# kuldeepbrd1/graspLDM

Measured on AMD Instinct MI355X. Metric: grasps/sec whole-node (1024-pt cloud, 100 DDIM steps), higher is better.
Workload: dtype f32 (GEMMs as split-f16 x3 partial products on the f16 matrix pipe, f32 accumulation; GroupNorm / LayerNorm / attention / scheduler in f32); 1 GPU; LDM mode, 256 synthetic 1024-pt clouds per GPU x 20 grasps, 100 DDIM steps: BASELINE.json configs[2] per GPU (configs[3] = this per-GPU workload on 8 GPUs); experiment=fpc, clouds_per_gpu=256, grasps_per_cloud=20, points=1024, ddim_steps=100, encoder=PVCNNEncoder (shipped fpc config), parallelism=cloud-sharded x1, weights=synthetic recipe seed 0, streams=3

## Files before the change

### graspldm_amd/_lib.py

```python
import ctypes
import os

_PKG = os.path.dirname(os.path.abspath(__file__))
LIB_PATH = os.environ.get("GLDM_LIB") or os.path.join(_PKG, "libgldm_hip.so")

ABI_VERSION = 10


class GldmError(RuntimeError):
    pass


_lib = None

_ll = ctypes.c_longlong
_ull = ctypes.c_ulonglong
_vp, _i, _f = ctypes.c_void_p, ctypes.c_int, ctypes.c_float

_SIGNATURES = {
    "gldm_ball_query": [_vp, _vp, _i, _i, _i, _f, _i, _vp, _vp],
    "gldm_grouping_forward": [_vp, _vp, _i, _i, _i, _i, _i, _vp, _vp],
    "gldm_gather_features_forward": [_vp, _vp, _i, _i, _i, _i, _vp, _vp],
    "gldm_furthest_point_sampling": [_vp, _i, _i, _i, _vp, _vp],
    "gldm_three_nn_interpolate_forward": [_vp, _vp, _vp, _i, _i, _i, _i, _vp, _vp, _vp, _vp],
    "gldm_avg_voxelize_forward": [_vp, _vp, _i, _i, _i, _i, _vp, _vp, _vp, _vp],
    "gldm_trilinear_devoxelize_forward": [_vp, _vp, _i, _i, _i, _i, _i, _vp, _vp, _vp, _vp],
    "gldm_voxel_coords": [_vp, _i, _i, _i, _i, _f, _vp, _vp, _vp],
    "gldm_farthest_points_euclid": [_vp, _i, _i, _i, _vp, _vp],
    "gldm_normalize_cloud": [_vp, _i, _i, _f, _f, _f, _f, _f, _f, _vp, _vp, _vp],
    "gldm_gather_points": [_vp, _vp, _i, _i, _i, _vp, _vp],
    "gldm_sa_group": [_vp, _vp, _vp, _i, _i, _i, _i, _f, _i, _vp, _vp, _vp],
    "gldm_r1d_cond_embed": [_vp, _vp, _vp, _i, _i, _i, _i, _vp, _vp],
    "gldm_denoise": [_vp, _vp, _vp, _vp, _i, _vp, _i, _vp, _vp, _i, _i, _i, _vp, _vp, _vp, _vp, _vp, _vp],
    "gldm_denoise_rng": [_vp, _vp, _vp, _vp, _i, _vp, _i, _vp, _i, _i, _vp, _ull, _ll, _vp, _vp, _vp, _vp],
    "gldm_step_noise_rng": [_ull, _ll, _i, _i, _i, _vp, _vp],
    "gldm_decode": [_vp, _vp, _vp, _i, _vp, _i, _vp, _vp, _vp, _vp],
    "gldm_pose_epilogue": [_vp, _vp, _vp, _vp, _i, _i, _i, _vp, _vp, _vp, _vp],
    "gldm_conv3d_k3": [_vp, _vp, _vp, _i, _i, _i, _i, _vp, _vp, _vp],
    "gldm_conv3d_k3_cl": [_vp, _vp, _vp, _i, _i, _i, _i, _vp, _vp, _vp],
    "gldm_conv3d_k3_generic": [_vp, _vp, _vp, _i, _i, _i, _i, _vp, _vp, _vp],
    "gldm_conv3d_k3_f16x2": [_vp, _vp, _vp, _i, _i, _i, _i, _vp, _vp, _vp],
    "gldm_conv3d_k3_f16x2_gn": [_vp, _vp, _vp, _vp, _i, _i, _i, _i, _vp, _vp, _i, _vp],
    "gldm_groupnorm_coef": [_vp, _vp, _vp, _i, _i, _i, _i, _f, _vp, _vp],
    "gldm_gn_swish_chan_sum": [_vp, _vp, _i, _i, _i, _vp, _vp],
    "gldm_gn_swish_chan_sum_cl": [_vp, _vp, _i, _i, _i, _vp, _vp],
    "gldm_se_gate_parts": [_vp, _i, _vp, _vp, _i, _i, _i, _i, _i, _vp, _vp],
    "gldm_groupnorm_swish": [_vp, _vp, _vp, _vp, _i, _i, _i, _i, _f, _vp, _vp],
    "gldm_se_gate": [_vp, _vp, _vp, _i, _i, _i, _i, _i, _vp, _vp],
    "gldm_bias_act": [_vp, _vp, _i, _i, ctypes.c_longlong, _i, _vp],
    "gldm_devoxelize_fused": [_vp, _vp, _vp, _vp, _i, _i, _i, _i, _vp, _vp],
    "gldm_devoxelize_gn_fused": [_vp, _vp, _vp, _vp, _vp, _i, _i, _i, _i, _vp, _vp],
    "gldm_devoxelize_gn_cl_fused": [_vp, _vp, _vp, _vp, _vp, _i, _i, _i, _i, _vp, _vp],
    "gldm_pointwise_mlp": [_vp, _vp, _vp, _i, _i, _i, _i, _i, _vp, _vp, _i, _vp, _vp, _vp],
    "gldm_pointwise_mlp2": [_vp, _vp, _vp, _i, _vp, _vp, _i, _i, _i, _i, _vp, _vp, _i, _vp, _vp, _vp],
    "gldm_pointwise_small": [_vp, _vp, _vp, _i, _i, _i, ctypes.c_longlong, _i, _vp, _vp],
    "gldm_pointwise_any": [_vp, _vp, _vp, _i, _i, _i, ctypes.c_longlong, _i, _vp, _vp],
    "gldm_linear_rows": [_vp, _vp, _vp, _i, _i, _i, _vp, _vp],
    "gldm_pointwise_mlp_f16x2": [_vp, _vp, _vp, _i, _i, _i, _i, _i, _vp, _vp, _i, _vp, _vp, _vp],
    "gldm_row_max": [_vp, _ll, _i, _vp, _vp],
    "gldm_pointwise_mlp_f16x2_pm": [_vp, _vp, _vp, _i, _i, _i, _i, _i, _vp, _vp],
    "gldm_pointwise_mlp_f16x2_add": [_vp, _vp, _vp, _vp, _ll, _ll, _ll, _i, _i, _i, _i, _i, _vp, _vp],
    "gldm_pointwise_mlp2_f16x2": [_vp, _vp, _vp, _i, _vp, _vp, _i, _i, _i, _i, _vp, _vp, _i, _vp, _vp, _vp, _vp],
    "gldm_sa_mlp_forward": [_vp, _vp, _vp, _vp, _vp, _i, _i, _i, _i, _i, _i, _vp, _vp, _vp, _vp, _vp, _vp],
    "gldm_sa_mlp_forward_f16x2": [_vp, _vp, _vp, _vp, _vp, _i, _i, _i, _i, _i, _i, _vp, _vp, _vp, _vp, _vp, _vp, _vp],
    "gldm_sa_mlp_forward_f16x2_pre": [_vp, _vp, _vp, _i, _vp, _vp, _i, _i, _i, _i, _i, _i, _vp, _vp, _vp, _vp, _vp, _vp, _vp],
}


# ... 61 lines not shown
```

### graspldm_amd/csrc/resnet1d.hip

```cpp
#include <hip/hip_runtime.h>
#include <type_traits>
#include <stdint.h>
#include <stdio.h>
#include <stdlib.h>

#include "gldm.h"
#include "wstream.h"
#include "devstate.h"

#define GLDM_API extern "C" __attribute__((visibility("default")))

#ifdef GLDM_DEBUG_KNOBS
#define GLDM_SKIP(c, bit) ((c).skip & (bit))
#define GLDM_STAMPS(p) (p)
#else
#define GLDM_SKIP(c, bit) false
#define GLDM_STAMPS(p) ((long long *)nullptr)
#endif

namespace {

using f32x4 = __attribute__((ext_vector_type(4))) float;
typedef __attribute__((address_space(3))) float lds_f;
typedef __attribute__((address_space(3))) f32x4 lds_f4;

constexpr int kHeads = 4, kDimHead = 32, kHidden = kHeads * kDimHead;
constexpr int kMaxC = 256;
constexpr int kMaxSegs = 64;

template <int NC>
struct Geo {
  static constexpr int kWaves = NC / 8;
  static constexpr int kThreads = kWaves * 64;
// ... 363 lines not shown
}


typedef __attribute__((ext_vector_type(8))) _Float16 f16x8;

__device__ __forceinline__ void split_planes8(const float (&x)[8], u32x4 (&pl)[kSplit]) {
#pragma unroll
  for (int q = 0; q < 4; ++q) {
    unsigned h, l;
    split_f16x2(x[2 * q], x[2 * q + 1], h, l);
    pl[0][q] = h;
    pl[1][q] = l;
  }
}
__device__ __forceinline__ f32x4 mfma_h(const u32x4 &a, const u32x4 &b, const f32x4 &c) {
  return __builtin_amdgcn_mfma_f32_16x16x32_f16(__builtin_bit_cast(f16x8, a), __builtin_bit_cast(f16x8, b), c, 0, 0, 0);
}
__device__ __forceinline__ f32x4 mfma_split(const u32x4 (&a)[kSplit], const u32x4 (&b)[kSplit], f32x4 acc) {
  acc = mfma_h(a[0], b[1], acc);
  acc = mfma_h(a[1], b[0], acc);
  return mfma_h(a[0], b[0], acc);
}

#if defined(GLDM_DEBUG_KNOBS) && defined(GLDM_EXP_NO_A)
constexpr bool kExpNoA = true;
#else
constexpr bool kExpNoA = false;
#endif
#if defined(GLDM_DEBUG_KNOBS) && defined(GLDM_EXP_NO_B)
constexpr bool kExpNoB = true;
#else
constexpr bool kExpNoB = false;
#endif
struct NoPreA { static constexpr bool on = false; };
template <int MT>
struct PreA {
  static constexpr bool on = true;
  static constexpr int kSets = MT == 1 ? 3 : 1;
  u32x4 a[kSets][MT][kSplit];
  __device__ __forceinline__ void request(const WStream &wv, int mt0, int cin) {
    const int kb32 = cin >> 5, kblocks = 3 * kb32;
#pragma unroll
    for (int t = 0; t < kSets; ++t)
#pragma unroll
      for (int mi = 0; mi < MT; ++mi)
#pragma unroll
        for (int pl = 0; pl < kSplit; ++pl) a[t][mi][pl] = wv.raw_at(((mt0 + mi) * kblocks + t * kb32) * kFragBytes, pl * 1024);
  }
};

template <int MT, int P0, int NP, class PRE = NoPreA>
__device__ __forceinline__ void gemm_pm3_pl(const Ctx &c, const float *__restrict__ wp3, int cin, int mt0,
                                            const float *planes, f32x4 (&acc)[MT][NP], const PRE &pre = PRE()) {
  constexpr int PB0 = P0 > 0 ? P0 - 1 : 0, PB1 = P0 + NP < 4 ? P0 + NP : 3, NB = PB1 - PB0 + 1;
  const int col = c.lane & 15, g = c.lane >> 4;
  const int kb32 = cin >> 5, kblocks = 3 * kb32;
  const WStream wv(wp3, c.lane);
  const lds_u4 *pl3 = (const lds_u4 *)planes + g * 64 + 16 * PB0 + col;
  constexpr int NA = MT == 1 ? 3 : 2;
  constexpr int NBUF = (MT == 1 && NB <= 3) ? 2 : 1;
  u32x4 a[NA][MT][kSplit];
  u32x4 bs[NBUF][NB][kSplit];
  auto load_a = [&](int buf, int t, int kb) {
    if (kExpNoA && kb > 0) return;
#pragma unroll
    for (int mi = 0; mi < MT; ++mi)
#pragma unroll
      for (int pl = 0; pl < kSplit; ++pl)
        a[buf][mi][pl] = wv.raw_at(((mt0 + mi) * kblocks + t * kb32 + kb) * kFragBytes, pl * 1024);
  };
  auto load_b = [&](int buf, int kb) {
    if (kExpNoB && kb > 0) return;
#pragma unroll
    for (int q = 0; q < NB; ++q)
#pragma unroll
      for (int pl = 0; pl < kSplit; ++pl) bs[buf][q][pl] = pl3[(kb * kSplit + pl) * 256 + 16 * q];
  };
  auto tap_mfmas = [&](int abuf, int bbuf, int t) {
#pragma unroll
    for (int mi = 0; mi < MT; ++mi)
// ... 131 lines not shown
        for (int st = 0; st < 6; ++st) step(st, kb0);
      }
    }
  } else {
    static_assert(MT == 1 || NT == 4, "two m-tiles per wave: all four tiles");
    u32x4 bs[2][kSplit];
    auto load_b1 = [&](int buf, int kb, int t, int q) {
#pragma unroll
      for (int pl = 0; pl < kSplit; ++pl) bs[buf][pl] = pl3[(kb * kSplit + pl) * G::kPlaneU4 + 16 * q + 4 * t];
    };
    first_a();
    load_b1(0, 0, 0, 0);
    auto step = [&](int st, int kb0) {
      const int t = st % 3, kb = kb0 + st / 3;
      const int nt = (st + 1) % 3, nkb0 = kb0 + (st + 1) / 3, nkb = nkb0 < last ? nkb0 : last;
      load_a((st + 1) & 1, nt, nkb);
#pragma unroll
      for (int q = 0; q < 4; ++q) {
        if (q < 3) load_b1((q + 1) & 1, kb, t, q + 1);
        else load_b1(0, nkb, nt, 0);
        __builtin_amdgcn_sched_barrier(0);
#pragma unroll
        for (int mi = 0; mi < MT; ++mi) acc[mi][q] = mfma_split(a[st & 1][mi], bs[q & 1], acc[mi][q]);
        __builtin_amdgcn_sched_barrier(0);
      }
    };
    for (int kb0 = 0; kb0 < kb32; kb0 += 2) {
#pragma unroll
      for (int st = 0; st < 6; ++st) step(st, kb0);
    }
  }
}

struct NoFirst { static constexpr bool on = false; };
struct Frag3 { static constexpr bool on = true; u32x4 p[kSplit]; };
template <int KB32, int MT, int NT, class PRE = NoPre, int MS = 1, int LL = 4, class FIRST = NoFirst>
__device__ __forceinline__ void gemm1_pl(const Ctx &c, const float *__restrict__ wp3, int mt0, int nt0, const float *planes,
                                         f32x4 (&acc)[MT][NT], const PRE &pre = PRE(), const FIRST &first = FIRST()) {
  const int col = c.lane & 15, g = c.lane >> 4;
  const WStream wv(wp3, c.lane);
  using PGx = PG<LL>;
  const lds_u4 *pl3 = (const lds_u4 *)planes + g * PGx::kCols + PGx::kOff + 16 * nt0 + col;
  u32x4 a[2][MT][kSplit];
  u32x4 bs[2][kSplit];
  auto load_a = [&](int buf, int kb) {
#pragma unroll
    for (int mi = 0; mi < MT; ++mi) {
      const int sb = ((mt0 + mi * MS) * KB32 + kb) * kFragBytes;
#pragma unroll
      for (int pl = 0; pl < kSplit; ++pl) a[buf][mi][pl] = wv.raw_at(sb, pl * 1024);
    }
  };
  auto load_b = [&](int buf, int kb, int ni) {
#pragma unroll
    for (int pl = 0; pl < kSplit; ++pl) bs[buf][pl] = pl3[(kb * kSplit + pl) * PGx::kPlaneU4 + 16 * ni];
  };
  if constexpr (FIRST::on) {
#pragma unroll
    for (int pl = 0; pl < kSplit; ++pl) a[0][0][pl] = first.p[pl];
    if constexpr (MT > 1) {
#pragma unroll
      for (int mi = 1; mi < MT; ++mi) {
        const int sb = ((mt0 + mi * MS) * KB32) * kFragBytes;
#pragma unroll
        for (int pl = 0; pl < kSplit; ++pl) a[0][mi][pl] = wv.raw_at(sb, pl * 1024);
      }
    }
  } else {
    load_a(0, 0);
  }
  load_b(0, 0, 0);
  __builtin_amdgcn_sched_barrier(0);
  pre();
  __builtin_amdgcn_sched_barrier(0);
#pragma unroll
  for (int kb = 0; kb < KB32; ++kb) {
    if (kb + 1 < KB32) load_a((kb + 1) & 1, kb + 1);
    __builtin_amdgcn_sched_barrier(0);
#pragma unroll
    for (int ni = 0; ni < NT; ++ni) {
      const int step = kb * NT + ni, nxt = step + 1;
      if (nxt < KB32 * NT) load_b(nxt & 1, nxt / NT, nxt % NT);
      __builtin_amdgcn_sched_barrier(0);
#pragma unroll
      for (int mi = 0; mi < MT; ++mi) acc[mi][ni] = mfma_split(a[kb & 1][mi], bs[step & 1], acc[mi][ni]);
      __builtin_amdgcn_sched_barrier(0);
    }
  }
}

// ... 327 lines not shown
  const int sm = LL == 16 ? (c.lane & 3) : cl;
  f32x4 acc[MT][NP];
  const bool has_ss = FIN == 1 && g.ss_w >= 0;
  const bool ss_tab = LL == 16 && has_ss && c.ss_lane != nullptr;
  const int ekb = g.E >> 4;
  const WStream wss(c.w + (has_ss ? g.ss_w : 0), c.lane);
  f32x4 ga[MT], be[MT], sc[MT], sh[MT], a_sc[MT], a_sh[MT];
  auto load_params = [&]() {
#pragma unroll
    for (int mi = 0; mi < MT; ++mi) {
      const int mt = mt0 + mi, row0 = 16 * mt + 4 * kq;
      ga[mi] = *reinterpret_cast<const f32x4 *>(c.w + g.gamma_off + row0);
      be[mi] = *reinterpret_cast<const f32x4 *>(c.w + g.beta_off + row0);
      sc[mi] = f32x4{1.f, 1.f, 1.f, 1.f};
      sh[mi] = f32x4{0.f, 0.f, 0.f, 0.f};
      if (ss_tab) {
        sc[mi] = *reinterpret_cast<const f32x4 *>(c.ss_lane + g.tab_off + row0);
        sh[mi] = *reinterpret_cast<const f32x4 *>(c.ss_lane + g.tab_off + g.C + row0);
      } else if (has_ss) {
        const float *sb = c.w + g.ss_b;
        sc[mi] = *reinterpret_cast<const f32x4 *>(sb + row0);
        sh[mi] = *reinterpret_cast<const f32x4 *>(sb + g.C + row0);
        a_sc[mi] = wss[(size_t)mt * ekb * 64];
        a_sh[mi] = wss[(size_t)((g.C >> 4) + mt) * ekb * 64];
      }
    }
  };
  lds_f *hsc = (lds_f *)(c.lds + GG::kMiscHs);
  float hs = 1.0f;
  if constexpr (FIN == 2) hs = hsc[sm];
#pragma unroll
  for (int mi = 0; mi < MT; ++mi) {
    f32x4 bv = f32x4{0.f, 0.f, 0.f, 0.f};
    if (bias) bv = *reinterpret_cast<const f32x4 *>(bias + 16 * (mt0 + mi) + 4 * kq);
    if constexpr (FIN == 2) {
      const float hinv = __builtin_amdgcn_rcpf(hs);
#pragma unroll
      for (int r = 0; r < 4; ++r) bv[r] *= hinv;
    }
#pragma unroll
    for (int p = 0; p < NP; ++p) acc[mi][p] = bv;
  }
  GLDM_WV_STAMP(c, 0, (long long)__builtin_readcyclecounter());
  GLDM_WV_STAMP(c, 3, (long long)(cin * 1000 + cout));
  const bool src_is_x = src == c.lds + GG::kBufX;
  const float *bplanes = c.lds + (cin > kPlaneMaxC ? PGx::kW : (src_is_x ? PGx::kX : PGx::kH));
  if constexpr (LL == 16) gemm_sm3_pl<MT, P0, NP, PRE>(c, wp, cin, mt0, bplanes, acc, pre);
  else gemm_pm3_pl<MT, P0, NP, PRE>(c, wp, cin, mt0, bplanes, acc, pre);
  GLDM_WV_STAMP(c, 1, (long long)__builtin_readcyclecounter());
  if (FIN != 0) load_params();
  constexpr bool kWide = MT == 2;
  constexpr bool kPark = kWide && LL == 16;
  f32x4 *pk = reinterpret_cast<f32x4 *>(c.park) + (size_t)(c.wave * MT * NP) * 64 + c.lane;
  f32x4 parked[FIN == 2 && kPark ? MT : 1][FIN == 2 && kPark ? NP : 1];
  if constexpr (FIN == 2 && kPark) {
#pragma unroll
    for (int mi = 0; mi < MT; ++mi)
#pragma unroll
      for (int p = 0; p < NP; ++p) parked[mi][p] = pk[(mi * NP + p) * 64];
  }
  hook();
  if constexpr (FIN == 0) {
    if (alias) __syncthreads();
    if (live) {
      lds_f *d3 = (lds_f *)dst;
#pragma unroll
      for (int mi = 0; mi < MT; ++mi)
// ... 347 lines not shown
#pragma unroll
    for (int co = 0; co < 4; ++co) {
      float acc = cw.b[co];
#pragma unroll
      for (int ci = 0; ci < 4; ++ci) {
        const f32x4 wr = cw.wt[4 * ci + co];
        acc += wr[0] * lft[ci];
        acc += wr[1] * in[ci];
        acc += wr[2] * rgt[ci];
      }
      out[co] = acc;
    }
  };
  auto gn_act = [&](float (&v)[4], const ConvW &cw, bool ss) {
#pragma unroll
    for (int co = 0; co < 4; ++co) {
      const float m = half_sum(row_pair_sum(v[co])) * 0.25f;
      const float d = v[co] - m;
      const float rs = __builtin_amdgcn_rsqf(half_sum(row_pair_sum(d * d)) * 0.25f + 1e-5f);
      float y = d * rs * cw.g[co] + cw.be[co];
      if (ss) y = y * sc[co] + sh[co];
      v[co] = silu(y);
    }
  };
  float y[4], z[4];
  conv3(x, k1, y);
  gn_act(y, k1, true);
  conv3(y, k2, z);
  gn_act(z, k2, false);
#pragma unroll
  for (int co = 0; co < 4; ++co) X[pswz(co, n)] = x[co] + z[co];
}

template <int NT, int NPW, bool FULL, int LL = 4, class FIRST = NoFirst>
__device__ __forceinline__ void out_ln_wave(const Ctx &c, const float *wp, const float *bias, int mt0, int nt0,
                                            bool active, int p0, const float *src, int cin, float *xres, int C,
                                            const float *gain, const FIRST &first = FIRST()) {
  using GG = Geo<64>;
  constexpr int NC = 64;
  const int kq = c.lane >> 4, col = c.lane & 15;
  f32x4 acc[1][NT];
  lds_f *red1 = (lds_f *)(c.lds + GG::kMiscRed1), *red2 = (lds_f *)(c.lds + GG::kMiscRed2);
  const int row0 = 16 * mt0 + 4 * kq;
  const int nloc = C < 16 ? C : 16;
  f32x4 gv = f32x4{0.f, 0.f, 0.f, 0.f};
  if (active) {
    const f32x4 bv = *reinterpret_cast<const f32x4 *>(bias + row0);
#pragma unroll
    for (int ni = 0; ni < NT; ++ni) acc[0][ni] = bv;
    gemm1_pl<kHidden / 32, 1, NT, NoPre, 1, LL, FIRST>(c, wp, mt0, nt0, c.lds + PG<LL>::kH, acc, NoPre(), first);
    gv = *reinterpret_cast<const f32x4 *>(gain + row0);
    const float inv_n = __builtin_amdgcn_rcpf((float)nloc);
#pragma unroll
    for (int ni = 0; ni < NT; ++ni) {
      float s1 = 0.f;
#pragma unroll
      for (int r = 0; r < 4; ++r) s1 += (FULL || row0 + r < C) ? acc[0][ni][r] : 0.f;
      s1 = half_sum(row_pair_sum(s1));
      const float ml = s1 * inv_n;
      float s2 = 0.f;
#pragma unroll
      for (int r = 0; r < 4; ++r) {
        const float d = (FULL || row0 + r < C) ? acc[0][ni][r] - ml : 0.f;
        s2 += d * d;
      }
      s2 = half_sum(row_pair_sum(s2));
      if (kq == 0) {
        red1[c.wave * NC + 16 * (nt0 + ni) + col] = s1;
        red2[c.wave * NC + 16 * (nt0 + ni) + col] = s2;
      }
    }
  }
  __syncthreads();
  if (active) {
    const float inv_c = __builtin_amdgcn_rcpf((float)C), inv_n = __builtin_amdgcn_rcpf((float)nloc);
    lds_f *x3 = (lds_f *)xres;
#pragma unroll
    for (int ni = 0; ni < NT; ++ni) {
      const int cc = 16 * (nt0 + ni) + col;
      float ps[NPW], pm[NPW], tot = 0.f;
#pragma unroll
      for (int q = 0; q < NPW; ++q) {
        ps[q] = red1[(p0 + q) * NC + cc];
        pm[q] = red2[(p0 + q) * NC + cc];
// ... 47 lines not shown

template <int RP>
__device__ __forceinline__ void column_stats8(const Ctx &c, const float *src, float inv_c) {
  constexpr int NC = 64;
  using GG = Geo<NC>;
  const lds_f *s3 = (const lds_f *)src;
  const int n = 8 * c.wave + (c.lane & 7), rp = c.lane >> 3;
  float v[RP], sum = 0.f;
#pragma unroll
  for (int i = 0; i < RP; ++i) {
    v[i] = s3[pswz(rp + 8 * i, n)];
    sum += v[i];
  }
  auto all_parts = [](float x) {
    x += dpp_mov<0x128>(x);
    return half_sum(row_pair_sum(x));
  };
  const float mean = all_parts(sum) * inv_c;
  float m2 = 0.f;
#pragma unroll
  for (int i = 0; i < RP; ++i) {
    const float d = v[i] - mean;
    m2 = fmaf(d, d, m2);
  }
  const float rstd = __builtin_amdgcn_rsqf(all_parts(m2) * inv_c + 1e-5f);
  if (rp == 0) {
    ((lds_f *)(c.lds + GG::kMiscRed1))[n] = mean;
    ((lds_f *)(c.lds + GG::kMiscRed2))[n] = rstd;
  }
}

constexpr int kAttExch = 512 * 64;
static_assert(kAttExch + 8 * 24 * 16 <= Geo<64>::kArena, "attention exchange slots");
template <int KB32>
__device__ __forceinline__ void qkv_att_pm(const Ctx &c, int w_off, int s_off, const float *src, int C) {
  constexpr int NC = 64;
  using GG = Geo<NC>;
  if (GLDM_SKIP(c, 8)) return;
  const int head = c.wave >> 1, half = c.wave & 1;
  const int mt0 = 2 * head + half;
  const int sm = c.lane & 15, kq = c.lane >> 4;
  f32x4 acc[3][4];
  if constexpr (KB32 == 0) {
    const int n = c.lane;
    const lds_f *s3 = (const lds_f *)src;
    float x[4];
#pragma unroll
    for (int ci = 0; ci < 4; ++ci) x[ci] = s3[pswz(ci, n)];
    const float mean = (x[0] + x[1] + x[2] + x[3]) * 0.25f;
    float vt = 0.f;
#pragma unroll
    for (int ci = 0; ci < 4; ++ci) {
      const float d = x[ci] - mean;
      vt += d * d;
    }
    const float rstd = __builtin_amdgcn_rsqf(vt * 0.25f + 1e-5f);
    lds_f *ysc = (lds_f *)(c.lds + GG::kMiscRed1);
#pragma unroll
    for (int k = 0; k < 4; ++k) ysc[64 * k + n] = (x[k] - mean) * rstd;
    const WStream wv(c.w + w_off, c.lane);
    f32x4 f[3];
#pragma unroll
    for (int t = 0; t < 3; ++t) f[t] = wv[(size_t)(mt0 + 8 * t) * 64];
    float b[4];
#pragma unroll
    for (int j = 0; j < 4; ++j) b[j] = ysc[64 * kq + 16 * j + sm];
#pragma unroll
    for (int t = 0; t < 3; ++t)
#pragma unroll
      for (int j = 0; j < 4; ++j)
        acc[t][j] = __builtin_amdgcn_mfma_f32_16x16x4f32(f[t][0], b[j], f32x4{0.f, 0.f, 0.f, 0.f}, 0, 0, 0);
  } else {
    const float *wp = c.w + w_off, *srow = c.w + s_off;
    f32x4 sv[3];
#pragma unroll
    for (int mi = 0; mi < 3; ++mi) sv[mi] = *reinterpret_cast<const f32x4 *>(srow + 16 * (mt0 + 8 * mi) + 4 * kq);
#pragma unroll
    for (int mi = 0; mi < 3; ++mi)
#pragma unroll
      for (int ni = 0; ni < 4; ++ni) acc[mi][ni] = f32x4{0.f, 0.f, 0.f, 0.f};
    const float inv_c = __builtin_amdgcn_rcpf((float)C);
    auto stats = [&]() { column_stats8<4 * KB32>(c, src, inv_c); };
    gemm1_pl<KB32, 3, 4, decltype(stats), 8>(c, wp, mt0, 0, c.lds + kPlaneX, acc, stats);
    __syncthreads();
    const lds_f *mean3 = (const lds_f *)(c.lds + GG::kMiscRed1), *rstd3 = (const lds_f *)(c.lds + GG::kMiscRed2);
#pragma unroll
    for (int ni = 0; ni < 4; ++ni) {
      const float rstd = rstd3[16 * ni + sm];
      const float mr = mean3[16 * ni + sm] * rstd;
#pragma unroll
      for (int mi = 0; mi < 3; ++mi)
#pragma unroll
        for (int r = 0; r < 4; ++r) acc[mi][ni][r] = acc[mi][ni][r] * rstd - mr * sv[mi][r];
    }
  }
  float kn[4][4];
#pragma unroll
  for (int r = 0; r < 4; ++r) {
    const float km = fmaxf(fmaxf(acc[1][0][r], acc[1][1][r]), fmaxf(acc[1][2][r], acc[1][3][r]));
    float ks = 0.f;
#pragma unroll
    for (int p = 0; p < 4; ++p) {
      kn[p][r] = fast_exp(acc[1][p][r] - km);
      ks += kn[p][r];
    }
    const float inv = __builtin_amdgcn_rcpf(ks);
#pragma unroll
    for (int p = 0; p < 4; ++p) kn[p][r] *= inv;
  }
  float qe[4][4], qm[4], qs[4];
#pragma unroll
  for (int p = 0; p < 4; ++p) {
    float m = fmaxf(fmaxf(acc[0][p][0], acc[0][p][1]), fmaxf(acc[0][p][2], acc[0][p][3]));
    m = half_max(row_pair_max(m));
    float sum = 0.f;
#pragma unroll
// ... 731 lines not shown
  for (int i = 0; i < 4; ++i) sv[i] = *reinterpret_cast<const f32x4 *>(srow + 16 * mtile(i) + 4 * g);
  const float svv[2] = {srow[16 * mtile(4) + p], srow[16 * mtile(5) + p]};
  __syncthreads();
  const lds_f *mean3 = (const lds_f *)(c.lds + GG::kMiscRed1), *rstd3 = (const lds_f *)(c.lds + GG::kMiscRed2);
  constexpr float kL2e = 1.44269504088896340736f;
#pragma unroll
  for (int e = 0; e < 2; ++e) {
    const int sm = s0 + e;
    {
      const float rstd = rstd3[4 * p + sm];
      const float mr = mean3[4 * p + sm] * rstd;
#pragma unroll
      for (int i = 0; i < 4; ++i)
#pragma unroll
        for (int r = 0; r < 4; ++r) acc[i][e][r] = (acc[i][e][r] * rstd - mr * sv[i][r]) * kL2e;
    }
#pragma unroll
    for (int r = 0; r < 4; ++r) {
      const float rstd = rstd3[4 * (4 * g + r) + sm];
      const float mr = mean3[4 * (4 * g + r) + sm] * rstd;
      acc[4][e][r] = acc[4][e][r] * rstd - mr * svv[0];
      acc[5][e][r] = acc[5][e][r] * rstd - mr * svv[1];
    }
    const f32x4 qa[2] = {acc[0][e], acc[1][e]}, ka[2] = {acc[2][e], acc[3][e]}, vt[2] = {acc[4][e], acc[5][e]};
    f32x4 o[2];
    quad16_attention_head(qa, ka, vt, o);
#pragma unroll
    for (int u = 0; u < 2; ++u)
      store_planes4<16>(c.lds + PGx::kH, kDimHead * h + 16 * u + 4 * g, 4 * p + sm, o[u][0], o[u][1], o[u][2], o[u][3]);
  }
  __syncthreads();
}


template <int NC, int L>
__device__ __forceinline__ void run_tape(const Ctx &c0, const gldm_r1d_desc &d, const int *tape, kernarg_int *ktape, int n_ops, int E, long long *stamps) {
#if defined(GLDM_DEBUG_KNOBS) && defined(GLDM_EXP_LDS_TAPE)
  constexpr bool KARG = false;
#else
  constexpr bool KARG = NC == 64;
#endif
  for (int op = 0; op < n_ops; ++op) {
    if (stamps && c0.tid == 0) stamps[op] = (long long)__builtin_readcyclecounter();
    Ctx c = c0;
    asm volatile("" : "+v"(c.tid), "+v"(c.lane));
    int o[kOpInts];
    read_op<KARG>(tape, ktape, op, o);
    if (o[0] == OP_CONV && o[5] * o[6] >= 128 * 128) __builtin_amdgcn_s_setprio(0);
    else __builtin_amdgcn_s_setprio(3);
    switch (o[0]) {
      case OP_CONV: {
        if constexpr (NC == 64) {
          if (o[7] & kFlagFused) {
            int q[kOpInts];
            read_op<KARG>(tape, ktape, op + 1, q);
            const GnEpilogue g1{1, o[8], o[9], o[10], o[11], E, o[6], o[6] / 4, c.lds + o[4], (o[7] >> kFlagTabShift) << 2};
            const GnEpilogue g2{2, q[8], q[9], -1, 0, E, q[6], q[6] / 4, c.lds + q[4], 0};
            resblock_pm<L == 16 ? 16 : 4>(c, o[1], o[2], q[1], q[2], c.lds + o[3], c.lds + o[4], o[6], g1, g2, stamps ? stamps + op + 1 : nullptr);
            ++op;
            break;
          }
        }
        const int mode = GLDM_SKIP(c, 1) ? 0 : (o[7] >> 9) & 3;
        const GnEpilogue g{mode, o[8], o[9], GLDM_SKIP(c, 16) ? -1 : o[10], o[11], E, o[6], o[6] / 4, c.lds + o[4],
                           (o[7] >> kFlagTabShift) << 2};
        conv_gemm<NC, L>(c, o[1], o[2], c.lds + o[3], o[5], o[7] & 255, c.lds + o[4], o[6], (o[7] & kFlagAlias) != 0, 0, g);
        break;
      }
      case OP_QUAD:
        if constexpr (NC == 64 && L == 4) {
          if (c.wave < 4)
            quad_narrow_levels(c, (kernarg_desc *)((__attribute__((address_space(4))) const char *)__builtin_amdgcn_kernarg_segment_ptr() +
                                                    offsetof(RunArgs, d)));
#if defined(GLDM_DEBUG_KNOBS) && defined(GLDM_QEXP_DUP)
          else if (GLDM_QEXP_DUP == 2)
            quad_narrow_levels(c, (kernarg_desc *)((__attribute__((address_space(4))) const char *)__builtin_amdgcn_kernarg_segment_ptr() +
                                                    offsetof(RunArgs, d)));
#else
          else quad_loader(c);
#endif
          __syncthreads();
        } else if constexpr (NC == 64 && L == 16) {
          kernarg_desc *dkp = (kernarg_desc *)((__attribute__((address_space(4))) const char *)__builtin_amdgcn_kernarg_segment_ptr() +
                                               offsetof(RunArgs, d));
          const float *sstab;
          if (c.ss_lane) {
            const unsigned long long pv = (unsigned long long)c.ss_lane;
            const unsigned lo = (unsigned)__builtin_amdgcn_readlane((int)(unsigned)pv, c.wave & 3);
            const unsigned hi = (unsigned)__builtin_amdgcn_readlane((int)(unsigned)(pv >> 32), c.wave & 3);
            sstab = (const float *)(((unsigned long long)hi << 32) | lo);
          } else {
            quad16_ss_rows(c, dkp);
            __syncthreads();
            sstab = c.lds + kQ16SsLds + (c.wave & 3) * kQ16SsRows;
          }
          if (c.wave < 4) quad16_narrow_levels<1>(c, dkp, sstab);
          else quad_loader<QStream16<1>>(c);
          __syncthreads();
          zero_plane_pads16(c.lds, c.tid);
        }
        break;
      case OP_RES4:
        if (!GLDM_SKIP(c, 8)) {
          if constexpr (NC == 64 && L == 4) resblock4_pm(c, o, E);
          else if constexpr (NC != 64) resblock4_valu<NC>(c, o, E);
        }
        if (o[11]) __syncthreads();
        break;
      case OP_QKVATT:
        if constexpr (NC == 64) {
          if (o[4] == 128) {
            int q[kOpInts];
            read_op<KARG>(tape, ktape, op + 1, q);
// ... 599 lines not shown
#endif
  const int S = nc / L;
  const int tiles = (n_samples + S - 1) / S;
  Plan p{tiles, slots, 1, 0, 1, n_steps};
  if (tiles <= slots) return p;
  if (tiles / slots + 2 > kMaxSegs) { p.grid = -1; return p; }
  p.grid = slots;
  p.rounds = tiles / slots;
  p.left = tiles - p.rounds * slots;
  if (p.left > 0) {
    int g = slots / p.left;
    if (g > 8) g = 8;
    if (g > n_steps) g = n_steps;
    if (n_steps > 4095) g = 1;
    if (!allow_chain) g = 1;
    p.chain = g < 1 ? 1 : g;
    p.seglen = (n_steps + p.chain - 1) / p.chain;
  }
  return p;
}

template <int NC, int L>
int launch_one(const RunArgs &a, int tiles, hipStream_t s) {
  size_t lds_bytes = (size_t)Geo<NC>::kLdsFloats * sizeof(float);
#ifdef GLDM_DEBUG_KNOBS
  if (getenv("GLDM_R1D_ONE_WG") && lds_bytes < 100 * 1024) lds_bytes = 100 * 1024;
#endif
  struct Tag {};
  gldm_dev::allow_dynamic_lds<Tag>(reinterpret_cast<const void *>(&r1d_kernel<NC, L>), (int)lds_bytes);
  hipLaunchKernelGGL((r1d_kernel<NC, L>), dim3(tiles), dim3(Geo<NC>::kThreads), lds_bytes, s, a);
  return hipGetLastError() == hipSuccess ? GLDM_OK : GLDM_ERR_LAUNCH;
}

int launch_r1d(const RunArgs &a_in, hipStream_t s) {
  const bool pm4 = pm_supported(&a_in.d), pm16 = !pm4 && pm16_supported(&a_in.d), pm = pm4 || pm16;
  const int L = a_in.d.seq_len, nc = pm ? 64 : engine_nc();
  const Plan pl = make_plan(a_in.n_samples, a_in.n_steps, L, nc, a_in.sched_kind != GLDM_SCHED_DPMPP);
  const int tiles = pl.grid;
  if (tiles <= 0) return GLDM_ERR_UNSUPPORTED;
  RunArgs a = a_in;
  a.slots = pl.slots; a.rounds = pl.rounds; a.left_tiles = pl.left; a.chain = pl.chain; a.seglen = pl.seglen;
  a.park = nullptr;
  a.pm_nops = 0;
  if (pm) {
    static_assert(8 * GLDM_R1D_MAX_LEVELS + 2 <= kPmMaxOps && sizeof(RunArgs) <= 4096, "64-column tape in the kernel arguments");
    bool use_quad = true;
#ifdef GLDM_DEBUG_KNOBS
    if (getenv("GLDM_R1D_NOQUAD")) use_quad = false;
#endif
    if (pm16 && !(a_in.ss_tab != nullptr || a_in.d.emb_dim == 64)) use_quad = false;
    a.pm_nops = build_tape<64>(a_in.d, a.pm_tape, use_quad);
    const WsLayout wl = ws_layout(&a_in.d, a_in.n_samples);
    if (wl.park_off >= 0) a.park = reinterpret_cast<float *>(reinterpret_cast<char *>(a_in.ws) + wl.park_off);
  }
  a.n_cus = cu_count();
#ifdef GLDM_DEBUG_KNOBS
  {
    const char *e = getenv("GLDM_R1D_SKIP");
    a.skip = e ? atoi(e) : 0;
    const char *g = getenv("GLDM_R1D_STAGGER_US");
    a.stagger_ticks = g ? atoi(g) * 100 : 0;
  }
  const bool stamp = getenv("GLDM_R1D_STAMP") != nullptr;
#else
  const bool stamp = false;
#endif
  static long long *dstamps = nullptr;
  if (stamp && !dstamps) (void)hipMalloc(&dstamps, (kMaxOps + 2) * sizeof(long long));
  a.stamps = stamp ? dstamps : nullptr;
  const int rc = pm4 ? launch_one<64, 4>(a, tiles, s)
                     : (pm16 ? launch_one<64, 16>(a, tiles, s)
                             : (L == 4 ? launch_one<kEngineNC, 4>(a, tiles, s) : launch_one<kEngineNC, 16>(a, tiles, s)));
  if (stamp) {
    static long long host[kMaxOps + 2];
    static const char *names[] = {"", "CONV", "RES4", "LN", "ATT", "QKVLN", "OUTLN", "QKVAT", "QUAD"};
    const bool quad = (pm4 || pm16) && a.pm_nops > 0 && a.pm_tape[0] == OP_QUAD;
    (void)hipDeviceSynchronize();
    (void)hipMemcpy(host, dstamps, sizeof(host), hipMemcpyDeviceToHost);
    int dims[GLDM_R1D_MAX_LEVELS + 1];
    for (int i = 0; i <= a.d.n_levels; ++i) dims[i] = a.d.dims[i];
    int op = 0;
    auto line = [&](int type, int C, int cout, int taps) {
      printf("op %3d %-5s C=%3d cout=%3d k=%d : %7lld clk\n", op, names[type], C, cout, taps, host[op + 1] - host[op]);
      ++op;
    };
    auto resblock = [&](int C) {
      if (C == 4 && a.d.seq_len == 4) line(2, C, C, 3);
      else { line(1, C, C, 3); line(1, C, C, 3); }
    };
    if (quad) line(8, dims[0], 128, 3);
    for (int lv = quad ? 3 : 0; lv < a.d.n_levels; ++lv) {
      const int C = dims[lv];
// ... 1146 lines not shown
  if (!weights || !cemb || !x_in || !x_out || !workspace || n_samples <= 0 || n_steps <= 0 || samples_per_cond <= 0 ||
      noise_base < 0)
    return GLDM_ERR_INVALID_ARG;
  if (desc->latent_dim != 0 || (temb && !timesteps)) return GLDM_ERR_INVALID_ARG;
  if (!sched_coef || ((unsigned long long)sched_coef & 15)) return GLDM_ERR_INVALID_ARG;
  RunArgs a{};
  a.d = *desc;
  a.weights = weights; a.temb = temb; a.cemb = cemb; a.semb = sample_emb; a.samples_per_cond = samples_per_cond;
  a.x_in = x_in; a.n_samples = n_samples; a.timesteps = timesteps; a.sample_t = nullptr; a.n_steps = n_steps;
  a.sched_kind = GLDM_SCHED_DDPM; a.clip_sample = clip_sample; a.sched_coef = sched_coef; a.step_noise = nullptr;
  a.noise_seed = noise_seed; a.noise_base = noise_base; a.noise_on = 1;
  a.out0 = x_out; a.out1 = nullptr; a.ws = reinterpret_cast<float *>(workspace);
  return launch_r1d(a, reinterpret_cast<hipStream_t>(stream));
}

__global__ void philox_normal_kernel(unsigned long long seed, long long base, int step, int n, int L, float *out) {
  const int i = blockIdx.x * blockDim.x + threadIdx.x;
  if (i >= n * L) return;
  const int gi = i / L, l = i - gi * L;
  const unsigned long long g = (unsigned long long)(base + gi);
  float z4[4];
  philox_normal4(seed, (unsigned)g, (unsigned)(g >> 32), (unsigned)(l >> 2), (unsigned)step, z4);
  out[i] = z4[l & 3];
}
GLDM_API int gldm_step_noise_rng(unsigned long long noise_seed, long long noise_base, int step, int n_samples, int seq_len,
                                 float *out, gldm_stream_t stream) {
  if (!out || n_samples <= 0 || seq_len <= 0 || step < 0 || noise_base < 0) return GLDM_ERR_INVALID_ARG;
  const int total = n_samples * seq_len;
  hipLaunchKernelGGL(philox_normal_kernel, dim3((total + 255) / 256), dim3(256), 0, reinterpret_cast<hipStream_t>(stream), noise_seed,
                     noise_base, step, n_samples, seq_len, out);
  return hipGetLastError() == hipSuccess ? GLDM_OK : GLDM_ERR_LAUNCH;
}

GLDM_API int gldm_decode(const gldm_r1d_desc *desc, const float *weights, const float *cemb, int samples_per_cond,
                         const float *z_h, int n_samples, float *tmrp, float *logit, void *workspace,
                         gldm_stream_t stream) {
  int st = validate(desc);
  if (st != GLDM_OK) return st;
  if (!weights || !cemb || !z_h || !tmrp || !logit || !workspace || n_samples <= 0 || samples_per_cond <= 0)
    return GLDM_ERR_INVALID_ARG;
  if (desc->latent_dim <= 0 || desc->n_head != 7) return GLDM_ERR_INVALID_ARG;
  RunArgs a{};
  a.d = *desc;
  a.weights = weights; a.temb = nullptr; a.cemb = cemb; a.samples_per_cond = samples_per_cond;
  a.x_in = z_h; a.n_samples = n_samples; a.n_steps = 1; a.sched_kind = GLDM_SCHED_NONE;
  a.out0 = tmrp; a.out1 = logit; a.ws = reinterpret_cast<float *>(workspace);
  const int rows = ss_table_rows(desc);
  if (rows > 0) {
    const long long off = ws_layout(desc, n_samples).ss_off;
    float *tab = reinterpret_cast<float *>(reinterpret_cast<char *>(workspace) + off);
    const int n_cond = (n_samples + samples_per_cond - 1) / samples_per_cond;
    hipLaunchKernelGGL(ss_table_kernel, dim3(n_cond), dim3(256), 0, reinterpret_cast<hipStream_t>(stream), *desc, weights,
                       cemb, rows, tab);
    if (hipGetLastError() != hipSuccess) return GLDM_ERR_LAUNCH;
    a.ss_tab = tab;
    a.ss_stride = rows;
  }
  return launch_r1d(a, reinterpret_cast<hipStream_t>(stream));
}

GLDM_API int gldm_pose_epilogue(const float *tmrp, const float *logit, const float *grasp_mean,
                                const float *grasp_std, int n, int grasps_per_cloud, int n_clouds, float *H,
                                float *tmrp_unnorm, float *confidence, gldm_stream_t stream) {
  if (!tmrp || !grasp_mean || !grasp_std || !H || !tmrp_unnorm || n <= 0 || grasps_per_cloud <= 0 || n_clouds <= 0)
    return GLDM_ERR_INVALID_ARG;
  if ((long long)n_clouds * grasps_per_cloud < (long long)n) return GLDM_ERR_INVALID_ARG;
// ... 333 lines not shown
```

### include/gldm.h

```cpp
#ifndef GLDM_H_
#define GLDM_H_

#include <stdint.h>

#ifdef __cplusplus
extern "C" {
#endif

typedef void *gldm_stream_t;

enum gldm_status {
  GLDM_OK = 0,
  GLDM_ERR_INVALID_ARG = -1,
  GLDM_ERR_LAUNCH = -2,
  GLDM_ERR_UNSUPPORTED = -3,
  GLDM_ERR_WORKSPACE = -4
};

int gldm_abi_version(void);
const char *gldm_status_string(int status);


int gldm_ball_query(const float *centers , const float *points ,
                    int b, int n, int m, float radius, int u,
// ... 89 lines not shown
  gldm_r1d_level lv[GLDM_R1D_MAX_LEVELS];
  int32_t final_w, final_b;
  int32_t latent_dim;
  int32_t in_w, in_b;
  int32_t head_w, head_b;
  int32_t n_head;
} gldm_r1d_desc;

enum gldm_sched_kind { GLDM_SCHED_NONE = 0, GLDM_SCHED_DDIM = 1, GLDM_SCHED_DDPM = 2, GLDM_SCHED_DPMPP = 3 };
#define GLDM_SCHED_COEF_STRIDE 8

int gldm_r1d_cond_embed(const float *z_cond , const float *w , const float *b ,
                        int n_cond, int rows, int dc, int e, float *cemb , gldm_stream_t stream);

#define GLDM_R1D_WS_ERROR 12
long long gldm_r1d_workspace_bytes(const gldm_r1d_desc *desc, int n_samples);

int gldm_r1d_tile_columns(const gldm_r1d_desc *desc);

int gldm_denoise(const gldm_r1d_desc *desc, const float *weights, const float *temb, const float *cemb,
                 int samples_per_cond, const float *x_in , int n_samples,
                 const int32_t *timesteps , const int32_t *sample_t, int n_steps,
                 int sched_kind, int clip_sample, const float *sched_coef ,
                 const float *step_noise, const float *sample_emb, float *x_out , void *workspace,
                 gldm_stream_t stream);

int gldm_denoise_rng(const gldm_r1d_desc *desc, const float *weights, const float *temb, const float *cemb,
                     int samples_per_cond, const float *x_in , int n_samples,
                     const int32_t *timesteps , int n_steps, int clip_sample,
                     const float *sched_coef , unsigned long long noise_seed, long long noise_base,
                     const float *sample_emb, float *x_out , void *workspace, gldm_stream_t stream);
int gldm_step_noise_rng(unsigned long long noise_seed, long long noise_base, int step, int n_samples, int seq_len,
                        float *out , gldm_stream_t stream);

int gldm_decode(const gldm_r1d_desc *desc, const float *weights, const float *cemb, int samples_per_cond,
                const float *z_h , int n_samples, float *tmrp , float *logit ,
                void *workspace, gldm_stream_t stream);

int gldm_pose_epilogue(const float *tmrp , const float *logit , const float *grasp_mean,
                       const float *grasp_std, int n, int grasps_per_cloud, int n_clouds, float *H ,
                       float *tmrp_unnorm , float *confidence , gldm_stream_t stream);

int gldm_sa_mlp_forward(const float *points , const float *centers ,
                        const float *features , const int32_t *idx ,
                        const float *weights, int b, int c, int n, int m, int u, int n_layers,
                        const int32_t *cin_pad, const int32_t *cout, const int32_t *w_off, const int32_t *b_off,
                        float *out , gldm_stream_t stream);

int gldm_sa_mlp_forward_f16x2(const float *points , const float *centers ,
                               const float *features , const int32_t *idx ,
                               const float *weights, int b, int c, int n, int m, int u, int n_layers,
                               const int32_t *cin_pad, const int32_t *cout, const int32_t *w3_off, const int32_t *b_off,
                               const float *range_gain ,
                               float *out , gldm_stream_t stream);

int gldm_sa_mlp_forward_f16x2_pre(const float *points , const float *centers ,
                                   const float *pre , int pre_broadcast,
                                   const int32_t *idx , const float *weights,
                                   int wa_off, int b, int n, int m, int u, int n_layers,
                                   const int32_t *cin_pad, const int32_t *cout, const int32_t *w3_off, const int32_t *b_off,
                                   const float *range_gain ,
                                   float *out , gldm_stream_t stream);

int gldm_pointwise_mlp(const float *x , const float *w_packed, const float *bias ,
                       int b, int cin, int cout, int n, int relu,
                       const float *head_w_packed, const float *head_bias , int hout,
// ... 94 lines not shown
```

Measured before the change: 313,800 grasps/s.

## Add specialized wide-level tape path that prefetches next-op weights and biases

Result: no change. 315,100 grasps/s (median of 6 runs) (+0.4%).

```diff
diff --git a/graspldm_amd/_lib.py b/graspldm_amd/_lib.py
--- a/graspldm_amd/_lib.py
+++ b/graspldm_amd/_lib.py
@@ -34,6 +34,7 @@
     "gldm_denoise": [_vp, _vp, _vp, _vp, _i, _vp, _i, _vp, _vp, _i, _i, _i, _vp, _vp, _vp, _vp, _vp, _vp],
     "gldm_denoise_rng": [_vp, _vp, _vp, _vp, _i, _vp, _i, _vp, _i, _i, _vp, _ull, _ll, _vp, _vp, _vp, _vp],
     "gldm_step_noise_rng": [_ull, _ll, _i, _i, _i, _vp, _vp],
+    "gldm_r1d_force_tape": [_i],
     "gldm_decode": [_vp, _vp, _vp, _i, _vp, _i, _vp, _vp, _vp, _vp],
     "gldm_pose_epilogue": [_vp, _vp, _vp, _vp, _i, _i, _i, _vp, _vp, _vp, _vp],
     "gldm_conv3d_k3": [_vp, _vp, _vp, _i, _i, _i, _i, _vp, _vp, _vp],
diff --git a/graspldm_amd/csrc/resnet1d.hip b/graspldm_amd/csrc/resnet1d.hip
--- a/graspldm_amd/csrc/resnet1d.hip
+++ b/graspldm_amd/csrc/resnet1d.hip
@@ -1,4 +1,5 @@
 #include <hip/hip_runtime.h>
+#include <atomic>
 #include <type_traits>
 #include <stdint.h>
 #include <stdio.h>
@@ -428,10 +429,11 @@
 #else
 constexpr bool kExpNoB = false;
 #endif
-struct NoPreA { static constexpr bool on = false; };
+struct NoPreA { static constexpr bool on = false; static constexpr bool kBias = false; };
 template <int MT>
 struct PreA {
   static constexpr bool on = true;
+  static constexpr bool kBias = false;
   static constexpr int kSets = MT == 1 ? 3 : 1;
   u32x4 a[kSets][MT][kSplit];
   __device__ __forceinline__ void request(const WStream &wv, int mt0, int cin) {
@@ -442,6 +444,16 @@
       for (int mi = 0; mi < MT; ++mi)
 #pragma unroll
         for (int pl = 0; pl < kSplit; ++pl) a[t][mi][pl] = wv.raw_at(((mt0 + mi) * kblocks + t * kb32) * kFragBytes, pl * 1024);
+  }
+};
+
+template <int MT>
+struct PreAB : PreA<MT> {
+  static constexpr bool kBias = true;
+  f32x4 bv[MT];
+  __device__ __forceinline__ void request_bias(const float *bias, int mt0, int kq) {
+#pragma unroll
+    for (int mi = 0; mi < MT; ++mi) bv[mi] = *reinterpret_cast<const f32x4 *>(bias + 16 * (mt0 + mi) + 4 * kq);
   }
 };
 
@@ -639,8 +651,11 @@
   }
 }
 
-struct NoFirst { static constexpr bool on = false; };
-struct Frag3 { static constexpr bool on = true; u32x4 p[kSplit]; };
+struct NoFirst { static constexpr bool on = false; static constexpr int kMt = 0; static constexpr bool kBias = false; };
+struct Frag3 { static constexpr bool on = true; static constexpr int kMt = 1; static constexpr bool kBias = false; u32x4 p[kSplit]; };
+struct Frag3B { static constexpr bool on = true; static constexpr int kMt = 1; static constexpr bool kBias = true; u32x4 p[kSplit]; f32x4 bv; };
+template <int M>
+struct FragM { static constexpr bool on = true; static constexpr int kMt = M; static constexpr bool kBias = false; u32x4 p[M][kSplit]; };
 template <int KB32, int MT, int NT, class PRE = NoPre, int MS = 1, int LL = 4, class FIRST = NoFirst>
 __device__ __forceinline__ void gemm1_pl(const Ctx &c, const float *__restrict__ wp3, int mt0, int nt0, const float *planes,
                                          f32x4 (&acc)[MT][NT], const PRE &pre = PRE(), const FIRST &first = FIRST()) {
@@ -662,7 +677,13 @@
 #pragma unroll
     for (int pl = 0; pl < kSplit; ++pl) bs[buf][pl] = pl3[(kb * kSplit + pl) * PGx::kPlaneU4 + 16 * ni];
   };
-  if constexpr (FIRST::on) {
+  if constexpr (FIRST::on && FIRST::kMt > 1) {
+    static_assert(FIRST::kMt == MT, "one set of first fragments per m-tile");
+#pragma unroll
+    for (int mi = 0; mi < MT; ++mi)
+#pragma unroll
+      for (int pl = 0; pl < kSplit; ++pl) a[0][mi][pl] = first.p[mi][pl];
+  } else if constexpr (FIRST::on) {
 #pragma unroll
     for (int pl = 0; pl < kSplit; ++pl) a[0][0][pl] = first.p[pl];
     if constexpr (MT > 1) {
@@ -1056,7 +1077,8 @@
 #pragma unroll
   for (int mi = 0; mi < MT; ++mi) {
     f32x4 bv = f32x4{0.f, 0.f, 0.f, 0.f};
-    if (bias) bv = *reinterpret_cast<const f32x4 *>(bias + 16 * (mt0 + mi) + 4 * kq);
+    if constexpr (PRE::kBias) bv = pre.bv[mi];
+    else if (bias) bv = *reinterpret_cast<const f32x4 *>(bias + 16 * (mt0 + mi) + 4 * kq);
     if constexpr (FIN == 2) {
       const float hinv = __builtin_amdgcn_rcpf(hs);
 #pragma unroll
@@ -1470,10 +1492,10 @@
   for (int co = 0; co < 4; ++co) X[pswz(co, n)] = x[co] + z[co];
 }
 
-template <int NT, int NPW, bool FULL, int LL = 4, class FIRST = NoFirst>
+template <int NT, int NPW, bool FULL, int LL = 4, class FIRST = NoFirst, class HOOK = NoHook>
 __device__ __forceinline__ void out_ln_wave(const Ctx &c, const float *wp, const float *bias, int mt0, int nt0,
                                             bool active, int p0, const float *src, int cin, float *xres, int C,
-                                            const float *gain, const FIRST &first = FIRST()) {
+                                            const float *gain, const FIRST &first = FIRST(), const HOOK &hook = HOOK()) {
   using GG = Geo<64>;
   constexpr int NC = 64;
   const int kq = c.lane >> 4, col = c.lane & 15;
@@ -1483,11 +1505,14 @@
   const int nloc = C < 16 ? C : 16;
   f32x4 gv = f32x4{0.f, 0.f, 0.f, 0.f};
   if (active) {
-    const f32x4 bv = *reinterpret_cast<const f32x4 *>(bias + row0);
+    f32x4 bv;
+    if constexpr (FIRST::kBias) bv = first.bv;
+    else bv = *reinterpret_cast<const f32x4 *>(bias + row0);
 #pragma unroll
     for (int ni = 0; ni < NT; ++ni) acc[0][ni] = bv;
     gemm1_pl<kHidden / 32, 1, NT, NoPre, 1, LL, FIRST>(c, wp, mt0, nt0, c.lds + PG<LL>::kH, acc, NoPre(), first);
     gv = *reinterpret_cast<const f32x4 *>(gain + row0);
+    hook();
     const float inv_n = __builtin_amdgcn_rcpf((float)nloc);
 #pragma unroll
     for (int ni = 0; ni < NT; ++ni) {
@@ -1601,8 +1626,9 @@
 
 constexpr int kAttExch = 512 * 64;
 static_assert(kAttExch + 8 * 24 * 16 <= Geo<64>::kArena, "attention exchange slots");
-template <int KB32>
-__device__ __forceinline__ void qkv_att_pm(const Ctx &c, int w_off, int s_off, const float *src, int C) {
+template <int KB32, class FIRST = NoFirst>
+__device__ __forceinline__ void qkv_att_pm(const Ctx &c, int w_off, int s_off, const float *src, int C,
+                                           const FIRST &first = FIRST()) {
   constexpr int NC = 64;
   using GG = Geo<NC>;
   if (GLDM_SKIP(c, 8)) return;
@@ -1650,7 +1676,7 @@
       for (int ni = 0; ni < 4; ++ni) acc[mi][ni] = f32x4{0.f, 0.f, 0.f, 0.f};
     const float inv_c = __builtin_amdgcn_rcpf((float)C);
     auto stats = [&]() { column_stats8<4 * KB32>(c, src, inv_c); };
-    gemm1_pl<KB32, 3, 4, decltype(stats), 8>(c, wp, mt0, 0, c.lds + kPlaneX, acc, stats);
+    gemm1_pl<KB32, 3, 4, decltype(stats), 8, 4, FIRST>(c, wp, mt0, 0, c.lds + kPlaneX, acc, stats, first);
     __syncthreads();
     const lds_f *mean3 = (const lds_f *)(c.lds + GG::kMiscRed1), *rstd3 = (const lds_f *)(c.lds + GG::kMiscRed2);
 #pragma unroll
@@ -2448,6 +2474,8 @@
   __syncthreads();
 }
 
+
+#include "wide_levels.h"
 
 template <int NC, int L>
 __device__ __forceinline__ void run_tape(const Ctx &c0, const gldm_r1d_desc &d, const int *tape, kernarg_int *ktape, int n_ops, int E, long long *stamps) {
@@ -2495,6 +2523,15 @@
 #else
           else quad_loader(c);
 #endif
+          if (o[1]) {
+            PreAB<1> first;
+            first.request(WStream(c.w + ktape[kOpInts * (op + 1) + 1], c.lane), c.wave, 128);
+            first.request_bias(c.w + ktape[kOpInts * (op + 1) + 2], c.wave, c.lane >> 4);
+            asm volatile("s_waitcnt lgkmcnt(0)\n\ts_barrier" ::: "memory");
+            wide_levels_pm4(c0, ktape, op, E, stamps, first);
+            op += kWideOps;
+            break;
+          }
           __syncthreads();
         } else if constexpr (NC == 64 && L == 16) {
           kernarg_desc *dkp = (kernarg_desc *)((__attribute__((address_space(4))) const char *)__builtin_amdgcn_kernarg_segment_ptr() +
@@ -3160,6 +3197,8 @@
   return hipGetLastError() == hipSuccess ? GLDM_OK : GLDM_ERR_LAUNCH;
 }
 
+std::atomic<int> g_force_tape{0};
+
 int launch_r1d(const RunArgs &a_in, hipStream_t s) {
   const bool pm4 = pm_supported(&a_in.d), pm16 = !pm4 && pm16_supported(&a_in.d), pm = pm4 || pm16;
   const int L = a_in.d.seq_len, nc = pm ? 64 : engine_nc();
@@ -3180,12 +3219,16 @@
     a.pm_nops = build_tape<64>(a_in.d, a.pm_tape, use_quad);
     const WsLayout wl = ws_layout(&a_in.d, a_in.n_samples);
     if (wl.park_off >= 0) a.park = reinterpret_cast<float *>(reinterpret_cast<char *>(a_in.ws) + wl.park_off);
+    if (pm4 && !g_force_tape.load(std::memory_order_relaxed) && a_in.semb == nullptr &&
+        wide_tape_matches(a_in.d, a.pm_tape, a.pm_nops))
+      a.pm_tape[1] = 1;
   }
   a.n_cus = cu_count();
 #ifdef GLDM_DEBUG_KNOBS
   {
     const char *e = getenv("GLDM_R1D_SKIP");
     a.skip = e ? atoi(e) : 0;
+    if (a.skip && a.pm_nops > 0) a.pm_tape[1] = 0;
     const char *g = getenv("GLDM_R1D_STAGGER_US");
     a.stagger_ticks = g ? atoi(g) * 100 : 0;
   }
@@ -4398,6 +4441,11 @@
   return hipGetLastError() == hipSuccess ? GLDM_OK : GLDM_ERR_LAUNCH;
 }
 
+GLDM_API int gldm_r1d_force_tape(int on) {
+  g_force_tape.store(on != 0, std::memory_order_relaxed);
+  return GLDM_OK;
+}
+
 GLDM_API int gldm_decode(const gldm_r1d_desc *desc, const float *weights, const float *cemb, int samples_per_cond,
                          const float *z_h, int n_samples, float *tmrp, float *logit, void *workspace,
                          gldm_stream_t stream) {
diff --git a/graspldm_amd/csrc/wide_levels.h b/graspldm_amd/csrc/wide_levels.h
--- /dev/null
+++ b/graspldm_amd/csrc/wide_levels.h
@@ -0,0 +1,139 @@
+#ifndef GLDM_WIDE_LEVELS_H_
+#define GLDM_WIDE_LEVELS_H_
+
+constexpr int kWideOps = 9;
+
+template <int MT, int C, class PRE1, class HOOK2>
+__device__ __forceinline__ void wide_resblock(const Ctx &c, const int (&o)[kOpInts], const int (&q)[kOpInts], int E, int mt0,
+                                              long long *stamp2, const PRE1 &pre1, const HOOK2 &hook2) {
+  using GG = Geo<64>;
+  float *X = c.lds + GG::kBufX, *H = c.lds + GG::kBufH;
+  const GnEpilogue g1{1, o[8], o[9], o[10], o[11], E, C, C / 4, H, (o[7] >> kFlagTabShift) << 2};
+  const GnEpilogue g2{2, q[8], q[9], -1, 0, E, C, C / 4, X, 0};
+  const float *wp2 = c.w + q[1];
+  PreAB<MT> pa;
+  const WStream wv2(wp2, c.lane);
+  auto ask = [&]() {
+    pa.request(wv2, mt0, C);
+    pa.request_bias(c.w + q[2], mt0, c.lane >> 4);
+  };
+  conv_pm3_wave<MT, 0, 4, 0, 1, PRE1, decltype(ask), 4>(c, c.w + o[1], c.w + o[2], mt0, X, C, H, C, false, g1, pre1, ask);
+  __syncthreads();
+  if (stamp2 && c.tid == 0) *stamp2 = (long long)__builtin_readcyclecounter();
+  conv_pm3_wave<MT, 0, 4, 0, 2, PreAB<MT>, HOOK2, 4>(c, wp2, c.w + q[2], mt0, H, C, X, C, false, g2, pa, hook2);
+}
+
+__device__ __forceinline__ void wide_levels_pm4(const Ctx &c0, kernarg_int *ktape, int op0, int E, long long *stamps,
+                                                const PreAB<1> &first) {
+  using GG = Geo<64>;
+  auto enter = [&](Ctx &c, int op) {
+    if (stamps && c0.tid == 0) stamps[op] = (long long)__builtin_readcyclecounter();
+    c = c0;
+    asm volatile("" : "+v"(c.tid), "+v"(c.lane));
+  };
+  auto w_off = [&](int op) { return ktape[kOpInts * op + 1]; };
+  auto b_off = [&](int op) { return ktape[kOpInts * op + 2]; };
+  Ctx c = c0;
+  int o[kOpInts], q[kOpInts];
+
+  PreAB<1> pb;
+  {
+    const int op = op0 + 1;
+    enter(c, op);
+    read_op<true>(nullptr, ktape, op, o);
+    read_op<true>(nullptr, ktape, op + 1, q);
+    __builtin_amdgcn_s_setprio(0);
+    auto ask_b = [&]() {
+      pb.request(WStream(c.w + w_off(op0 + 3), c.lane), c.wave, 128);
+      pb.request_bias(c.w + b_off(op0 + 3), c.wave, c.lane >> 4);
+    };
+    wide_resblock<1, 128>(c, o, q, E, c.wave, stamps ? stamps + op + 1 : nullptr, first, ask_b);
+    __syncthreads();
+  }
+  FragM<3> fq;
+  {
+    const int op = op0 + 3;
+    enter(c, op);
+    read_op<true>(nullptr, ktape, op, o);
+    read_op<true>(nullptr, ktape, op + 1, q);
+    __builtin_amdgcn_s_setprio(0);
+    auto ask_q = [&]() {
+      const WStream wv(c.w + w_off(op0 + 5), c.lane);
+#pragma unroll
+      for (int mi = 0; mi < 3; ++mi)
+#pragma unroll
+        for (int pl = 0; pl < kSplit; ++pl) fq.p[mi][pl] = wv.raw_at(((c.wave + 8 * mi) * 4) * kFragBytes, pl * 1024);
+    };
+    wide_resblock<1, 128>(c, o, q, E, c.wave, stamps ? stamps + op + 1 : nullptr, pb, ask_q);
+    __syncthreads();
+  }
+  PreAB<2> pd;
+  {
+    const int op = op0 + 5;
+    enter(c, op);
+    read_op<true>(nullptr, ktape, op, o);
+    read_op<true>(nullptr, ktape, op + 1, q);
+    __builtin_amdgcn_s_setprio(3);
+    Frag3B out_first;
+    {
+      const Frag3 f = out_ln_request(c, q[1]);
+#pragma unroll
+      for (int pl = 0; pl < kSplit; ++pl) out_first.p[pl] = f.p[pl];
+      out_first.bv = *reinterpret_cast<const f32x4 *>(c.w + q[2] + 16 * c.wave + 4 * (c.lane >> 4));
+    }
+    qkv_att_pm<4>(c, o[1], o[2], c.lds + GG::kBufX, 128, fq);
+    if (stamps && c0.tid == 0) stamps[op + 1] = (long long)__builtin_readcyclecounter();
+    auto ask_d = [&]() {
+      pd.request(WStream(c.w + w_off(op0 + 7), c.lane), 2 * c.wave, 128);
+      pd.request_bias(c.w + b_off(op0 + 7), 2 * c.wave, c.lane >> 4);
+    };
+    out_ln_wave<4, 8, true, 4, Frag3B>(c, c.w + q[1], c.w + q[2], c.wave, 0, true, 0, c.lds + kPlaneH, kHidden, c.lds + GG::kBufX,
+                                      128, c.w + q[7], out_first, ask_d);
+  }
+  PreAB<2> pe;
+  {
+    const int op = op0 + 7;
+    enter(c, op);
+    read_op<true>(nullptr, ktape, op, o);
+    __builtin_amdgcn_s_setprio(0);
+    const GnEpilogue g{0, o[8], o[9], o[10], o[11], E, 256, 64, c.lds + GG::kBufX, (o[7] >> kFlagTabShift) << 2};
+    auto ask_e = [&]() {
+      pe.request(WStream(c.w + w_off(op0 + 8), c.lane), 2 * c.wave, 256);
+      pe.request_bias(c.w + b_off(op0 + 8), 2 * c.wave, c.lane >> 4);
+    };
+    conv_pm3_wave<2, 0, 4, 0, 0, PreAB<2>, decltype(ask_e), 4>(c, c.w + o[1], c.w + o[2], 2 * c.wave, c.lds + GG::kBufX, 128,
+                                                               c.lds + GG::kBufX, 256, true, g, pd, ask_e);
+    __syncthreads();
+  }
+  {
+    const int op = op0 + 8;
+    enter(c, op);
+    read_op<true>(nullptr, ktape, op, o);
+    read_op<true>(nullptr, ktape, op + 1, q);
+    __builtin_amdgcn_s_setprio(0);
+    wide_resblock<2, 256>(c, o, q, E, 2 * c.wave, stamps ? stamps + op + 1 : nullptr, pe, NoHook());
+    __syncthreads();
+  }
+}
+
+inline bool wide_tape_matches(const gldm_r1d_desc &d, const int *tape, int n_ops) {
+  using GG = Geo<64>;
+  if (n_ops != kWideOps + 1 || tape[0] != OP_QUAD || d.seq_len != 4 || d.n_levels != 4 || d.dims[3] != 128 || d.dims[4] != 256)
+    return false;
+  auto t = [&](int op, int i) { return tape[kOpInts * op + i]; };
+  auto block = [&](int op, int C) {
+    return t(op, 0) == OP_CONV && (t(op, 7) & kFlagFused) && ((t(op, 7) >> 9) & 3) == 1 && (t(op, 7) & 255) == 3 &&
+           t(op, 2) >= 0 && t(op, 3) == GG::kBufX && t(op, 4) == GG::kBufH && t(op, 5) == C && t(op, 6) == C &&
+           t(op + 1, 0) == OP_CONV && ((t(op + 1, 7) >> 9) & 3) == 2 && t(op + 1, 2) >= 0 && t(op + 1, 3) == GG::kBufH &&
+           t(op + 1, 4) == GG::kBufX && t(op + 1, 5) == C && t(op + 1, 6) == C;
+  };
+  return block(1, 128) && block(3, 128) &&
+         t(5, 0) == OP_QKVATT && t(5, 3) == GG::kBufX && t(5, 4) == 128 &&
+         t(6, 0) == OP_OUTLN && t(6, 3) == kPlaneH && t(6, 4) == GG::kBufX && t(6, 5) == kHidden && t(6, 6) == 128 &&
+         t(7, 0) == OP_CONV && !(t(7, 7) & kFlagFused) && ((t(7, 7) >> 9) & 3) == 0 && (t(7, 7) & 255) == 3 &&
+         (t(7, 7) & kFlagAlias) && t(7, 2) >= 0 && t(7, 3) == GG::kBufX && t(7, 4) == GG::kBufX && t(7, 5) == 128 &&
+         t(7, 6) == 256 &&
+         block(8, 256);
+}
+
+#endif
diff --git a/include/gldm.h b/include/gldm.h
--- a/include/gldm.h
+++ b/include/gldm.h
@@ -145,6 +145,7 @@
                      const float *sample_emb, float *x_out , void *workspace, gldm_stream_t stream);
 int gldm_step_noise_rng(unsigned long long noise_seed, long long noise_base, int step, int n_samples, int seq_len,
                         float *out , gldm_stream_t stream);
+int gldm_r1d_force_tape(int on);
 
 int gldm_decode(const gldm_r1d_desc *desc, const float *weights, const float *cemb, int samples_per_cond,
                 const float *z_h , int n_samples, float *tmrp , float *logit ,
```
